# boundless-xyz/boundless

Measured on AMD Instinct MI355X. Metric: segment-proofs/sec @ 2^20 cycles, higher is better.
Workload: dtype u32 (BabyBear Montgomery)

## Files before the change

### boundless_amd/csrc/poseidon2.hip

```cpp
#include "ctx.hpp"
#include "poseidon2_arith.hpp"
#include "hash_suite.hpp"
#include "../../include/bx_image.h"

namespace bx {

constexpr int CELLS = 24, RATE = 16, RF_HALF = 4, RP = 21;
constexpr int DIAG_OFF = 216;
constexpr int PAIR_OFF = DIAG_OFF + 24, P2_TABLE = PAIR_OFF + 2 * CELLS;

typedef uint32_t sgpr8 __attribute__((ext_vector_type(8)));
static_assert(DIAG_OFF % 8 == 0 && PAIR_OFF % 8 == 0 && CELLS % 8 == 0, "the tables are read as 32-byte octets");
template <int LO = 0, int HI = CELLS>
__device__ __forceinline__ void poseidon2_mix(uint32_t* io, const uint32_t* __restrict__ prm) {
    i32 s[CELLS];
    i64 y[CELLS];
#pragma unroll
    for (int i = 0; i < CELLS; ++i) s[i] = (i32)io[i];
    m_ext64s(s, y);
    redc64s_all(y, prm, s);
#pragma unroll 1
    for (int r = 0; r < RF_HALF; ++r) {
        sbox7s_n<CELLS / 2>(s);
        sbox7s_n<CELLS / 2>(s + CELLS / 2);
        m_ext64s(s, y);
        if (r < RF_HALF - 1) {
            redc64s_all(y, prm + (r + 1) * CELLS, s);
        } else {
            red64ks_all<K1_MID, K2_MID, true>(y, prm[96], s);
        }
    }
    {
        const sgpr8* kp = reinterpret_cast<const sgpr8*>(prm + PAIR_OFF);
        sgpr8 k0 = kp[0], k1 = kp[1], k2 = kp[2], k3 = kp[3], k4 = kp[4], k5 = kp[5];
        asm volatile("" : "+s"(k0), "+s"(k1), "+s"(k2), "+s"(k3), "+s"(k4), "+s"(k5));
        i32 pk[2 * CELLS];
#pragma unroll
        for (int i = 0; i < 8; ++i) {
            pk[i] = (i32)k0[i], pk[8 + i] = (i32)k1[i], pk[16 + i] = (i32)k2[i];
            pk[24 + i] = (i32)k3[i], pk[32 + i] = (i32)k4[i], pk[40 + i] = (i32)k5[i];
        }
#pragma unroll 1
        for (int r = 0; r < RP - 1; r += 2) {
            internal_round_pair(s, pk, pk + CELLS, prm + 97 + r);
        }
    }
    uint32_t diag[CELLS];
    {
        const sgpr8* dp = reinterpret_cast<const sgpr8*>(prm + DIAG_OFF);
        sgpr8 d0 = dp[0], d1 = dp[1], d2 = dp[2];
        asm volatile("" : "+s"(d0), "+s"(d1), "+s"(d2));
#pragma unroll
        for (int i = 0; i < 8; ++i) diag[i] = d0[i], diag[8 + i] = d1[i], diag[16 + i] = d2[i];
    }
    internal_round<true>(s, diag, prm + 117);
    i64 t[4];
#pragma unroll 1
    for (int r = 0;; ++r) {
        sbox7s_n<CELLS / 2>(s);
        sbox7s_n<CELLS / 2>(s + CELLS / 2);
        m_ext64s_core(s, y, t);
        asm volatile("" : "+s"(r));
        if (r == RF_HALF - 1) break;
        m_ext64s_finish(y, t);
        redc64s_all(y, prm + 117 + (r + 1) * CELLS, s);
    }
    m_ext64s_finish<LO, HI>(y, t);
    red64ks_all<K1_END, K2_END, false, LO, HI>(y, 0u, s);
#pragma unroll
    for (int i = LO; i < HI; ++i) io[i] = canon(s[i]);
}

__global__ __launch_bounds__(256) __attribute__((amdgpu_waves_per_eu(4, 4))) void hash_rows_kernel(uint32_t* __restrict__ out, const uint32_t* __restrict__ matrix,
                                                        const uint32_t* __restrict__ prm, uint32_t rows, uint32_t cols) {
    uint32_t r = blockIdx.x * blockDim.x + threadIdx.x;
    if (r >= rows) return;
    uint32_t s[CELLS];
#pragma unroll
    for (int i = 0; i < CELLS; ++i) s[i] = 0u;
    const uint32_t* p = matrix + r;
    uint32_t c = 0;
    for (; c + RATE < cols; c += RATE) {
#pragma unroll
        for (int i = 0; i < RATE; ++i) s[i] = p[(size_t)(c + i) * rows];
        poseidon2_mix<RATE, CELLS>(s, prm);
    }
#pragma unroll
    for (int i = 0; i < RATE; ++i) s[i] = (c + i < cols) ? p[(size_t)(c + i) * rows] : 0u;
    poseidon2_mix<0, 8>(s, prm);
    uint4* o = reinterpret_cast<uint4*>(out + (size_t)r * 8);
    o[0] = make_uint4(s[0], s[1], s[2], s[3]);
    o[1] = make_uint4(s[4], s[5], s[6], s[7]);
}

__global__ __launch_bounds__(256) __attribute__((amdgpu_waves_per_eu(4, 4))) void hash_fold_kernel(uint32_t* __restrict__ io, const uint32_t* __restrict__ prm,
                                                        uint32_t input_size, uint32_t output_size) {
    uint32_t i = blockIdx.x * blockDim.x + threadIdx.x;
    if (i >= output_size) return;
    const uint4* src = reinterpret_cast<const uint4*>(io + ((size_t)input_size + 2 * (size_t)i) * 8);
    uint32_t s[CELLS];
    uint4 v0 = src[0], v1 = src[1], v2 = src[2], v3 = src[3];
    s[0] = v0.x; s[1] = v0.y; s[2] = v0.z; s[3] = v0.w;
    s[4] = v1.x; s[5] = v1.y; s[6] = v1.z; s[7] = v1.w;
    s[8] = v2.x; s[9] = v2.y; s[10] = v2.z; s[11] = v2.w;
    s[12] = v3.x; s[13] = v3.y; s[14] = v3.z; s[15] = v3.w;
#pragma unroll
    for (int k = 16; k < CELLS; ++k) s[k] = 0u;
    poseidon2_mix<0, 8>(s, prm);
    uint4* o = reinterpret_cast<uint4*>(io + ((size_t)output_size + i) * 8);
    o[0] = make_uint4(s[0], s[1], s[2], s[3]);
    o[1] = make_uint4(s[4], s[5], s[6], s[7]);
}

__global__ __launch_bounds__(256) __attribute__((amdgpu_waves_per_eu(4, 4))) void hash_fold_indexed_kernel(uint32_t* out, const uint32_t* in,
                                                                const uint32_t* __restrict__ sel, const uint32_t* __restrict__ prm,
                                                                uint32_t count, uint32_t n_in) {
    uint32_t j = blockIdx.x * blockDim.x + threadIdx.x;
    if (j >= count) return;
    uint2 pr = reinterpret_cast<const uint2*>(sel)[j];
    pr.x = pr.x < n_in ? pr.x : n_in - 1;
    pr.y = pr.y < n_in ? pr.y : n_in - 1;
    const uint4* a = reinterpret_cast<const uint4*>(in + (size_t)pr.x * 8);
    const uint4* b = reinterpret_cast<const uint4*>(in + (size_t)pr.y * 8);
    uint32_t s[CELLS];
    uint4 v0 = a[0], v1 = a[1], v2 = b[0], v3 = b[1];
    s[0] = v0.x; s[1] = v0.y; s[2] = v0.z; s[3] = v0.w;
    s[4] = v1.x; s[5] = v1.y; s[6] = v1.z; s[7] = v1.w;
    s[8] = v2.x; s[9] = v2.y; s[10] = v2.z; s[11] = v2.w;
    s[12] = v3.x; s[13] = v3.y; s[14] = v3.z; s[15] = v3.w;
#pragma unroll
    for (int k = 16; k < CELLS; ++k) s[k] = 0u;
    poseidon2_mix<0, 8>(s, prm);
    uint4* o = reinterpret_cast<uint4*>(out + (size_t)j * 8);
    o[0] = make_uint4(s[0], s[1], s[2], s[3]);
    o[1] = make_uint4(s[4], s[5], s[6], s[7]);
}

__device__ __forceinline__ void fold_pair(uint32_t* out8, const uint32_t* a8, const uint32_t* b8, const uint32_t* __restrict__ prm) {
    uint32_t s[CELLS];
#pragma unroll
    for (int k = 0; k < 8; ++k) s[k] = a8[k], s[8 + k] = b8[k];
#pragma unroll
    for (int k = 16; k < CELLS; ++k) s[k] = 0u;
    uint32_t z;
    asm volatile("s_mov_b32 %0, 0" : "=s"(z));
    poseidon2_mix<0, 8>(s, prm + z);
#pragma unroll
    for (int k = 0; k < 8; ++k) out8[k] = s[k];
}
__device__ __forceinline__ void ld_digest(uint32_t* d, const uint32_t* p) {
    const uint4 a = reinterpret_cast<const uint4*>(p)[0], b = reinterpret_cast<const uint4*>(p)[1];
    d[0] = a.x; d[1] = a.y; d[2] = a.z; d[3] = a.w; d[4] = b.x; d[5] = b.y; d[6] = b.z; d[7] = b.w;
}
__device__ __forceinline__ void st_digest(uint32_t* p, const uint32_t* d) {
    reinterpret_cast<uint4*>(p)[0] = make_uint4(d[0], d[1], d[2], d[3]);
    reinterpret_cast<uint4*>(p)[1] = make_uint4(d[4], d[5], d[6], d[7]);
}
template <int LVL>
__device__ __forceinline__ void fold_subtree(uint32_t* out8, uint32_t* __restrict__ io, const uint32_t* __restrict__ prm, size_t input_size, size_t idx) {
    uint32_t a[8], b[8];
    if constexpr (LVL == 1) {
        ld_digest(a, io + (input_size + 2 * idx) * 8);
        ld_digest(b, io + (input_size + 2 * idx + 1) * 8);
    } else {
        fold_subtree<LVL - 1>(a, io, prm, input_size, 2 * idx);
        fold_subtree<LVL - 1>(b, io, prm, input_size, 2 * idx + 1);
    }
    fold_pair(out8, a, b, prm);
// ... 153 lines not shown
        sbox7s_n<QS>(s);
        m_ext_quad(s, y, m);
        if (r < RF_HALF - 1) redc_quad(y, shp + 117 + (r + 1) * CELLS + q, s);
        else redk_quad<K1_END, K2_END>(y, 0u, s);
    }
#pragma unroll
    for (int k = 0; k < QS; ++k) io[k] = canon(s[k]);
}

__global__ __launch_bounds__(1024) void hash_fold_quad_kernel(uint32_t* __restrict__ io, const uint32_t* __restrict__ prm, uint32_t input_size,
                                                              uint32_t per_wg, int levels) {
    __shared__ uint32_t sh[256 * 8];
    __shared__ uint32_t shp[DIAG_OFF + 24];
    const uint32_t tid = threadIdx.x, q = tid & 3, node = tid >> 2;
    for (uint32_t i = tid; i < DIAG_OFF + 24; i += blockDim.x) shp[i] = prm[i];
    uint32_t width = per_wg >> 1;
    uint32_t out_size = input_size >> 1;
    for (int lvl = 0; lvl < levels; ++lvl) {
        const bool active = node < width;
        uint32_t s[QS];
        if (active) {
            if (lvl == 0) {
                const uint32_t* src = io + ((size_t)input_size + 2 * ((size_t)blockIdx.x * width + node)) * 8;
#pragma unroll
                for (int k = 0; k < 4; ++k) s[k] = src[4 * k + q];
            } else {
#pragma unroll
                for (int k = 0; k < 4; ++k) s[k] = sh[node * 16 + 4 * k + q];
            }
            s[4] = 0u;
            s[5] = 0u;
        }
        __syncthreads();
        if (active) {
            poseidon2_mix_quad(s, shp, q);
            uint32_t* o = io + ((size_t)out_size + (size_t)blockIdx.x * width + node) * 8;
            o[q] = s[0];
            o[4 + q] = s[1];
            sh[node * 8 + q] = s[0];
            sh[node * 8 + 4 + q] = s[1];
        }
        __syncthreads();
        width >>= 1;
        out_size >>= 1;
    }
}

__global__ __launch_bounds__(64) void transcript_step_kernel(uint32_t* __restrict__ state, const uint32_t* __restrict__ digests, uint32_t n_commit,
                                                            uint32_t* __restrict__ out, uint32_t n_elems, const uint32_t* __restrict__ prm) {
    __shared__ uint32_t shp[DIAG_OFF + 24];
    const uint32_t tid = threadIdx.x, q = tid & 3;
    for (uint32_t i = tid; i < DIAG_OFF + 24; i += blockDim.x) shp[i] = prm[i];
    __syncthreads();
    if (tid >= 4) return;
    uint32_t s[QS];
#pragma unroll
    for (int k = 0; k < QS; ++k) s[k] = state[4 * k + q];
    uint32_t pool = state[24];
    for (uint32_t i = 0; i < n_commit; ++i) {
        if (pool != 0) {
            poseidon2_mix_quad(s, shp, q);
            pool = 0;
        }
        s[0] = fp_add(s[0], digests[8 * i + q]);
        s[1] = fp_add(s[1], digests[8 * i + 4 + q]);
        poseidon2_mix_quad(s, shp, q);
    }
    for (uint32_t e = 0; e < n_elems; ++e) {
        if (pool == 16) {
            poseidon2_mix_quad(s, shp, q);
            pool = 0;
        }
        const uint32_t slot = pool >> 2;
        const uint32_t v = slot == 0 ? s[0] : slot == 1 ? s[1] : slot == 2 ? s[2] : s[3];
        if ((pool & 3u) == q) out[e] = v;
        ++pool;
    }
#pragma unroll
    for (int k = 0; k < QS; ++k) state[4 * k + q] = s[k];
    if (q == 0) state[24] = pool;
}

const char* poseidon2_upload_params(bx_ctx* c) {
    uint32_t h[P2_TABLE] = {0};
    for (int i = 0; i < 213; ++i) h[i] = (uint32_t)((uint64_t)(c->h_rc[i] % P) * p2_rc_scale(i) % P);
    for (int i = 0; i < 24; ++i) h[DIAG_OFF + i] = fp_encode(c->h_diag[i]);
    i32 pe[CELLS], pa[CELLS];
    p2_pair_consts(h + DIAG_OFF, pe, pa);
    for (int i = 0; i < CELLS; ++i) h[PAIR_OFF + i] = (uint32_t)pe[i], h[PAIR_OFF + CELLS + i] = (uint32_t)pa[i];
    if (!c->d_p2) BX_HIP(c, hipMalloc(&c->d_p2, sizeof h));
    BX_HIP(c, hipMemcpyAsync(c->d_p2, h, sizeof h, hipMemcpyHostToDevice, c->stream));
    BX_HIP(c, stream_wait(c));
    return nullptr;
}

static const char* launch_hash_rows(bx_ctx* c, uint32_t* out, const uint32_t* matrix, size_t rows, size_t cols) {
    if (rows == 0) return nullptr;
    unsigned bs = (unsigned)c->hash_rows_block;
    hipLaunchKernelGGL(hash_rows_kernel, dim3((unsigned)((rows + bs - 1) / bs)), dim3(bs), 0, c->stream, out, matrix, c->d_p2,
                       (uint32_t)rows, (uint32_t)cols);
    BX_LAUNCH_CHECK(c);
    return nullptr;
}
static const char* launch_hash_fold(bx_ctx* c, uint32_t* io, size_t input_size, size_t output_size) {
    if (output_size == 0) return nullptr;
    hipLaunchKernelGGL(hash_fold_kernel, dim3((unsigned)((output_size + 255) / 256)), dim3(256), 0, c->stream, io, c->d_p2,
                       (uint32_t)input_size, (uint32_t)output_size);
    BX_LAUNCH_CHECK(c);
    return nullptr;
}
template <int L>
static const char* launch_hash_fold_deep(bx_ctx* c, uint32_t* io, size_t size) {
    hipLaunchKernelGGL(hash_fold_deep_kernel<L>, dim3((unsigned)(((size >> L) + 255) / 256)), dim3(256), 0, c->stream, io, c->d_p2, (uint32_t)size);
    BX_LAUNCH_CHECK(c);
    return nullptr;
}
static const char* launch_hash_fold_small(bx_ctx* c, uint32_t* io, size_t size, size_t per_wg, int levels) {
    if (c->fold_quad)
        hipLaunchKernelGGL(hash_fold_quad_kernel, dim3((unsigned)(size / per_wg)), dim3((unsigned)(2 * per_wg)), 0, c->stream, io, c->d_p2,
                           (uint32_t)size, (uint32_t)per_wg, levels);
    else
        hipLaunchKernelGGL(hash_fold_multi_kernel, dim3((unsigned)(size / per_wg)), dim3(256), 0, c->stream, io, c->d_p2, (uint32_t)size,
                           (uint32_t)per_wg, levels);
    BX_LAUNCH_CHECK(c);
    return nullptr;
}
HashLaunchers poseidon2_launchers() { return {launch_hash_rows, launch_hash_fold, launch_hash_fold_deep<3>, launch_hash_fold_deep<2>, launch_hash_fold_small}; }

}

using namespace bx;

extern "C" const char* bx_poseidon2_set_params(bx_ctx* c, const uint32_t* rc213, const uint32_t* diag24) try {
    if (!c) return "bx_poseidon2_set_params: null ctx";
    BX_REQUIRE(c, rc213 && diag24, "poseidon2_set_params: null table");
    BX_REQUIRE(c, c->live_provers == 0, "poseidon2_set_params: destroy the provers of this ctx first (their transcripts hold the old table)");
    BX_ENTER(c);
    for (int i = 0; i < 213; ++i) c->h_rc[i] = rc213[i] % P;
    for (int i = 0; i < 24; ++i) c->h_diag[i] = diag24[i] % P;
    return poseidon2_upload_params(c);
} BX_ABI_CATCH(c, "bx_poseidon2_set_params")
extern "C" const char* bx_poseidon2_get_params(bx_ctx* c, uint32_t* rc213, uint32_t* diag24) try {
    if (!c) return "bx_poseidon2_get_params: null ctx";
    for (int i = 0; i < 213; ++i) rc213[i] = c->h_rc[i];
    for (int i = 0; i < 24; ++i) diag24[i] = c->h_diag[i];
    return nullptr;
} BX_ABI_CATCH(c, "bx_poseidon2_get_params")

extern "C" const char* bx_hash_fold_indexed(bx_ctx* c, bx_buf out, bx_buf in, bx_buf sel, size_t count) try {
    if (!c) return "bx_hash_fold_indexed: null ctx";
    BX_REQUIRE(c, count <= out.len / 8 && count <= sel.len / 2, "hash_fold_indexed: out or sel too small");
    BX_REQUIRE(c, count <= 0xffffffffu && in.len / 8 <= 0xffffffffu, "hash_fold_indexed: too many digests");
    if (count == 0) return nullptr;
    BX_REQUIRE(c, out.dptr && in.dptr && sel.dptr && in.len >= 8, "hash_fold_indexed: null or empty buffer");
    BX_REQUIRE(c, !bufs_overlap(out, in), "hash_fold_indexed: out and in overlap");
    BX_REQUIRE(c, !bufs_overlap(out, sel), "hash_fold_indexed: out and sel overlap");
    BX_ENTER(c);
    OpScope op(c, "hash_fold_indexed", 104.0 * (double)count);
    hipLaunchKernelGGL(hash_fold_indexed_kernel, dim3((unsigned)((count + 255) / 256)), dim3(256), 0, c->stream, (uint32_t*)out.dptr,
                       (const uint32_t*)in.dptr, (const uint32_t*)sel.dptr, c->d_p2, (uint32_t)count, (uint32_t)(in.len / 8));
    BX_LAUNCH_CHECK(c);
    return nullptr;
} BX_ABI_CATCH(c, "bx_hash_fold_indexed")

extern "C" const char* bx_transcript_step(bx_ctx* c, bx_buf state, bx_buf digests, size_t n_commit, bx_buf out_ext, size_t n_ext) try {
    if (!c) return "bx_transcript_step: null ctx";
    BX_REQUIRE(c, c->hash_suite == SUITE_POSEIDON2, "transcript_step: the device transcript is Poseidon2's (a sha-256 ctx draws on the host)");
    BX_REQUIRE(c, state.dptr != nullptr && state.len >= 25, "transcript_step: the state is 24 cells and the pool counter");
    BX_REQUIRE(c, n_commit <= 64 && n_ext <= 64, "transcript_step: at most 64 commits and 64 challenges per step");
    BX_REQUIRE(c, digests.len >= 8 * n_commit && out_ext.len >= 4 * n_ext, "transcript_step: digests / out too small");
    BX_REQUIRE(c, !bufs_overlap(out_ext, state), "transcript_step: out_ext and state overlap");
    BX_REQUIRE(c, !bufs_overlap(out_ext, digests), "transcript_step: out_ext and digests overlap");
// ... 9 lines not shown
```

### boundless_amd/csrc/poseidon2_arith.hpp

```cpp
#pragma once
#include "fp.hpp"

#if defined(BX_CHECK_BOUNDS) && !defined(__HIP_DEVICE_COMPILE__)
#include <stdio.h>
#include <stdlib.h>
#define BX_ASSERT_BOUND(cond, what)                                              \
    do {                                                                         \
        if (!(cond)) {                                                           \
            fprintf(stderr, "bound violated: %s (%s:%d)\n", what, __FILE__, __LINE__); \
            abort();                                                             \
        }                                                                        \
    } while (0)
#else
#define BX_ASSERT_BOUND(cond, what) ((void)0)
#endif

#if defined(BX_PLAIN_MAD)
#define BX_MAD_FLAVOUR mad_plain
#else
#define BX_MAD_FLAVOUR mad_pinned
#endif
namespace bx {
inline namespace BX_MAD_FLAVOUR {

constexpr int P2_CELLS = 24;

constexpr uint32_t cx_mul(uint32_t a, uint32_t b) { return (uint32_t)((uint64_t)a * b % P); }
constexpr uint32_t cx_pow(uint32_t b, uint64_t e) {
    uint32_t r = 1;
    while (e) {
        if (e & 1) r = cx_mul(r, b);
        b = cx_mul(b, b);
        e >>= 1;
    }
    return r;
}
constexpr uint32_t cx_rpow(int64_t e) { return cx_pow(MONT_ONE, e >= 0 ? (uint64_t)e : (uint64_t)((int64_t)(P - 1) + e)); }
constexpr uint32_t K1_MID = cx_rpow(2801), K2_MID = cx_mul(K1_MID, MONT_ONE);
constexpr uint32_t K1_END = cx_rpow(400), K2_END = cx_mul(K1_END, MONT_ONE);
constexpr uint32_t p2_rc_scale(int i) {
    return i < 24 ? cx_rpow(1) : i < 48 ? cx_rpow(-6) : i < 72 ? cx_rpow(-55) : i < 96 ? cx_rpow(-398)
         : i < 141 ? cx_rpow(2)
         : i < 165 ? cx_rpow(1) : i < 189 ? cx_rpow(-6) : cx_rpow(-55);
}

using i32 = int32_t;
using i64 = int64_t;
constexpr i64 SREDC_MAX = ((i64)0x7fffffff - (i64)(P / 2) - 2) * ((i64)1 << 32);

#if defined(__HIP_DEVICE_COMPILE__) && !defined(BX_PLAIN_MAD)
#define BX_MAD_ASM(op, args, ...)                                                                  \
    do {                                                                                           \
        switch (alt & 3) {                                                                         \
            case 0: asm volatile(op " %0, s[40:41], " args : "=v"(r) : __VA_ARGS__ : "s40", "s41"); break; \
            case 1: asm volatile(op " %0, s[42:43], " args : "=v"(r) : __VA_ARGS__ : "s42", "s43"); break; \
            case 2: asm volatile(op " %0, s[44:45], " args : "=v"(r) : __VA_ARGS__ : "s44", "s45"); break; \
            default: asm volatile(op " %0, s[46:47], " args : "=v"(r) : __VA_ARGS__ : "s46", "s47"); break; \
        }                                                                                          \
    } while (0)
#endif
BX_HD i64 smad(i32 a, i32 b, i64 c, int alt = 0) {
#if defined(__HIP_DEVICE_COMPILE__) && !defined(BX_PLAIN_MAD)
    i64 r;
    BX_MAD_ASM("v_mad_i64_i32", "%1, %2, %3", "v"(a), "v"(b), "v"(c));
    return r;
#else
    (void)alt;
    return (i64)a * (i64)b + c;
#endif
}
BX_HD i64 smul(i32 a, i32 b, int alt = 0) {
#if defined(__HIP_DEVICE_COMPILE__) && !defined(BX_PLAIN_MAD)
    i64 r;
    BX_MAD_ASM("v_mad_i64_i32", "%1, %2, 0", "v"(a), "v"(b));
    return r;
#else
    (void)alt;
    return (i64)a * (i64)b;
#endif
}
BX_HD i64 smad_k(i32 a, uint32_t k, i64 c, int alt = 0) {
#if defined(__HIP_DEVICE_COMPILE__) && !defined(BX_PLAIN_MAD)
    i64 r;
    BX_MAD_ASM("v_mad_i64_i32", "%1, %2, %3", "v"(a), "s"(k), "v"(c));
    return r;
#else
    (void)alt;
    return (i64)a * (i64)k + c;
#endif
}
BX_HD i64 smul_k(i32 a, uint32_t k, int alt = 0) {
#if defined(__HIP_DEVICE_COMPILE__) && !defined(BX_PLAIN_MAD)
    i64 r;
    BX_MAD_ASM("v_mad_i64_i32", "%1, %2, 0", "v"(a), "s"(k));
    return r;
#else
    (void)alt;
    return (i64)a * (i64)k;
#endif
}
BX_HD i64 smad_s(i32 a, i32 k, i64 c, int alt = 0) {
#if defined(__HIP_DEVICE_COMPILE__) && !defined(BX_PLAIN_MAD)
    i64 r;
    BX_MAD_ASM("v_mad_i64_i32", "%1, %2, %3", "v"(a), "s"(k), "v"(c));
    return r;
#else
    (void)alt;
    return (i64)a * (i64)k + c;
#endif
}
BX_HD i64 smul_s(i32 a, i32 k, int alt = 0) {
#if defined(__HIP_DEVICE_COMPILE__) && !defined(BX_PLAIN_MAD)
    i64 r;
    BX_MAD_ASM("v_mad_i64_i32", "%1, %2, 0", "v"(a), "s"(k));
    return r;
#else
    (void)alt;
    return (i64)a * (i64)k;
#endif
}
template <int K>
BX_HD i64 smadc(i32 a, i64 c, int alt = 0) {
#if defined(__HIP_DEVICE_COMPILE__) && !defined(BX_PLAIN_MAD)
    i64 r;
    BX_MAD_ASM("v_mad_i64_i32", "%1, %3, %2", "v"(a), "v"(c), "n"(K));
    return r;
#else
    (void)alt;
    return (i64)a * K + c;
#endif
}
template <int K>
BX_HD i64 smulc(i32 a, int alt = 0) {
#if defined(__HIP_DEVICE_COMPILE__) && !defined(BX_PLAIN_MAD)
    i64 r;
    BX_MAD_ASM("v_mad_i64_i32", "%1, %2, 0", "v"(a), "n"(K));
    return r;
#else
    (void)alt;
    return (i64)a * K;
#endif
}
BX_HD i64 add_u32(i64 c, uint32_t k, int alt = 0) {
#if defined(__HIP_DEVICE_COMPILE__) && !defined(BX_PLAIN_MAD)
    i64 r;
    BX_MAD_ASM("v_mad_u64_u32", "%1, 1, %2", "s"(k), "v"(c));
    return r;
#else
    (void)alt;
    return c + (i64)k;
#endif
}
BX_HD i64 umul_k(uint32_t a, uint32_t k, int alt = 0) {
#if defined(__HIP_DEVICE_COMPILE__) && !defined(BX_PLAIN_MAD)
    i64 r;
    BX_MAD_ASM("v_mad_u64_u32", "%1, %2, 0", "v"(a), "s"(k));
    return r;
#else
    (void)alt;
    return (i64)((uint64_t)a * (uint64_t)k);
#endif
}
BX_HD i32 mont_m(i64 t) {
#if defined(__HIP_DEVICE_COMPILE__) && !defined(BX_PLAIN_MAD)
    i32 m;
    asm volatile("v_mul_lo_u32 %0, %1, %2" : "=v"(m) : "v"((uint32_t)t), "s"(NEG_P_INV));
    return m;
#else
    return (i32)((uint32_t)t * NEG_P_INV);
#endif
}
BX_HD i32 sredc(i64 t, int alt = 0) {
    BX_ASSERT_BOUND(t <= SREDC_MAX && t >= -SREDC_MAX, "sredc operand");
    const i32 m = mont_m(t);
    return (i32)(smad_k(m, P, t, alt) >> 32);
}
BX_HD i64 iabs64(i64 v) { return v < 0 ? -v : v; }

constexpr i64 ub(i64 T) { return (T >> 32) + (i64)(P / 2) + 1; }
constexpr i64 B_IN = (i64)P - 1;
constexpr i64 B_Y = 112 * ((i64)1 << 31);
constexpr i64 B_EXT = ub(B_Y + (i64)P);
constexpr i64 B_MIDOUT = ub(((i64)1 << 32) * K1_MID + ((B_Y >> 32) + 1) * (i64)K2_MID + 2 * (i64)P);
constexpr i64 B_SUMR = ub(((i64)1 << 31) * R2 + 33 * (i64)R3);
constexpr i64 B_INT = (i64)((double)P * 0.945);
static_assert(ub((i64)(P - 1) * B_INT + B_SUMR + (i64)P) <= B_INT && B_MIDOUT <= B_INT, "internal-round bound is not invariant");
static_assert((i64)(P - 1) * B_INT + B_SUMR + (i64)P <= SREDC_MAX && B_INT * B_INT <= SREDC_MAX, "internal-round products overflow sredc");
static_assert(24 * B_INT < ((i64)1 << 37), "internal sum");

BX_HD uint64_t mad64(uint32_t a, uint32_t b, uint64_t c) { return (uint64_t)a * (uint64_t)b + c; }

template <int N>
BX_HD void sredc_n(const i64* t, i32* r) {
    i32 m[N];
#pragma unroll
    for (int i = 0; i < N; ++i) {
        BX_ASSERT_BOUND(t[i] <= SREDC_MAX && t[i] >= -SREDC_MAX, "sredc operand");
        m[i] = mont_m(t[i]);
    }
#pragma unroll
    for (int i = 0; i < N; ++i) r[i] = (i32)(smad_k(m[i], P, t[i], i & 3) >> 32);
}

BX_HD i32 sbox7s(i32 x) {
    BX_ASSERT_BOUND(iabs64(x) <= B_INT, "sbox input");
    const i32 x2 = sredc(smul(x, x));
    const i32 x3 = sredc(smul(x2, x));
    const i32 x4 = sredc(smul(x2, x2));
    return sredc(smul(x3, x4));
}
template <int N>
BX_HD void sbox7s_n(i32* x) {
    i64 t[N], u[N];
    i32 x2[N], x3[N], x4[N];
#pragma unroll
    for (int i = 0; i < N; ++i) {
        BX_ASSERT_BOUND(iabs64(x[i]) <= B_INT, "sbox input");
        t[i] = smul(x[i], x[i], i & 3);
    }
    sredc_n<N>(t, x2);
#pragma unroll
    for (int i = 0; i < N; ++i) {
        t[i] = smul(x2[i], x[i], 2 * i);
        u[i] = smul(x2[i], x2[i], 2 * i + 1);
    }
    sredc_n<N>(t, x3);
    sredc_n<N>(u, x4);
#pragma unroll
    for (int i = 0; i < N; ++i) t[i] = smul(x3[i], x4[i], i & 3);
    sredc_n<N>(t, x);
}

BX_HD i32 redc64s(i64 y, uint32_t rc) {
    BX_ASSERT_BOUND(iabs64(y) <= B_Y, "external layer output");
    const i32 r = sredc(add_u32(y, rc));
    BX_ASSERT_BOUND(iabs64(r) <= B_EXT, "redc64s output");
    return r;
}

BX_HD void redc64s_all(const i64* y, const uint32_t* rc, i32* s) {
    constexpr int H = P2_CELLS / 2;
#pragma unroll
    for (int h = 0; h < P2_CELLS; h += H) {
        i64 acc[H];
#pragma unroll
        for (int i = 0; i < H; ++i) {
            BX_ASSERT_BOUND(iabs64(y[h + i]) <= B_Y, "external layer output");
            acc[i] = add_u32(y[h + i], rc[h + i], i & 3);
        }
        sredc_n<H>(acc, s + h);
    }
#pragma unroll
    for (int i = 0; i < P2_CELLS; ++i) BX_ASSERT_BOUND(iabs64(s[i]) <= B_EXT, "redc64s output");
}

template <uint32_t K1, uint32_t K2, bool HAS_ADD = true>
BX_HD i32 red64ks(i64 y, uint32_t add) {
    BX_ASSERT_BOUND(iabs64(y) <= B_Y, "external layer output");
    static_assert(K1 < (1u << 29) && K2 < P, "correction constant too large for the accumulator bound");
    i64 acc = umul_k((uint32_t)y, K1);
    if (HAS_ADD) acc = add_u32(acc, add);
    return sredc(smad_k((i32)(y >> 32), K2, acc));
}
template <uint32_t K1, uint32_t K2, bool HAS_ADD0, int LO = 0, int HI = P2_CELLS>
BX_HD void red64ks_all(const i64* y, uint32_t add0, i32* s) {
    static_assert(K1 < (1u << 29) && K2 < P, "correction constant too large for the accumulator bound");
    static_assert(0 <= LO && LO < HI && HI <= P2_CELLS && (!HAS_ADD0 || LO == 0), "live range");
    constexpr int H = HI - LO < P2_CELLS / 2 ? HI - LO : P2_CELLS / 2;
    static_assert((HI - LO) % H == 0, "live range: a whole number of stages");
#pragma unroll
    for (int h = LO; h < HI; h += H) {
        i64 acc[H];
#pragma unroll
        for (int i = 0; i < H; ++i) {
            BX_ASSERT_BOUND(iabs64(y[h + i]) <= B_Y, "external layer output");
            acc[i] = umul_k((uint32_t)y[h + i], K1, i & 3);
        }
        if (HAS_ADD0 && h == 0) acc[0] = add_u32(acc[0], add0, 0);
#pragma unroll
        for (int i = 0; i < H; ++i) acc[i] = smad_k((i32)(y[h + i] >> 32), K2, acc[i], (i + 1) & 3);
        sredc_n<H>(acc, s + h);
    }
}

BX_HD void m_ext64s_core(const i32* s, i64* y, i64* t) {
#pragma unroll
    for (int h = 0; h < 2; ++h) {
        i64 t0[3], t1[3], t2[3], t3[3];
#pragma unroll
        for (int q = 0; q < 3; ++q) {
            const int g = 3 * h + q;
            t0[q] = smulc<1>(s[4 * g], 2 * q);
            t1[q] = smulc<1>(s[4 * g + 2], 2 * q + 1);
        }
#pragma unroll
        for (int q = 0; q < 3; ++q) {
            const int g = 3 * h + q;
            t0[q] = smadc<1>(s[4 * g + 1], t0[q], 2 * q + 2);
            t1[q] = smadc<1>(s[4 * g + 3], t1[q], 2 * q + 3);
        }
#pragma unroll
        for (int q = 0; q < 3; ++q) {
            const int g = 3 * h + q;
            t2[q] = smadc<2>(s[4 * g + 1], t1[q], 2 * q);
            t3[q] = smadc<2>(s[4 * g + 3], t0[q], 2 * q + 1);
        }
#pragma unroll
        for (int q = 0; q < 3; ++q) {
            const int g = 3 * h + q;
            const i64 t4 = t1[q] * 4 + t3[q], t5 = t0[q] * 4 + t2[q];
            y[4 * g] = t3[q] + t5;
            y[4 * g + 1] = t5;
            y[4 * g + 2] = t2[q] + t4;
            y[4 * g + 3] = t4;
        }
    }
#pragma unroll
    for (int j = 0; j < 4; ++j) {
        t[j] = y[j];
#pragma unroll
        for (int k = 4; k < P2_CELLS; k += 4) t[j] += y[k + j];
    }
}
template <int LO = 0, int HI = P2_CELLS>
BX_HD void m_ext64s_finish(i64* y, const i64* t) {
    static_assert(0 <= LO && LO < HI && HI <= P2_CELLS, "live range");
#pragma unroll
    for (int i = LO; i < HI; ++i) y[i] += t[i & 3];
}
BX_HD void m_ext64s(const i32* s, i64* y) {
    i64 t[4];
    m_ext64s_core(s, y, t);
    m_ext64s_finish(y, t);
}

BX_HD i32 internal_sum_rs(i64 sum) {
// ... 124 lines not shown
    i64 a0 = smul_s(x0, E[0], 2);
    i64 f = fold64(sum1, 3);
    gx = smad_s(s[2], A[2], gx, 0);
    m = mont_m(f);
    gy = smad_s(s[6], A[6], gy, 1);
    const i32 sig1 = (i32)(smad_k(m, P, f, 2) >> 32);
    BX_ASSERT_BOUND(iabs64(sig1) <= B_SIG1, "sig1");
    gx = smad_s(s[3], A[3], gx, 3);
    gy = smad_s(s[7], A[7], gy, 0);
    a0 = smad_k(sig1, R2, a0, 1);
    gx = smad_s(s[4], A[4], gx, 2);
    a0 = add_u32(a0, rc[0], 3);
    BX_ASSERT_BOUND(iabs64(a0) <= T_PAIR0, "cell 0, round A");
    gy = smad_s(s[8], A[8], gy, 0);
    m = mont_m(a0);
    gx = smad_s(sig1, K23R3, gx, 1);
    const i32 y0 = (i32)(smad_k(m, P, a0, 2) >> 32);
    BX_ASSERT_BOUND(iabs64(y0) <= B_INT && iabs64(gx) <= T_DOT && iabs64(gy) <= T_DOT, "sbox input");
    i64 fx = fold64(gx, 3);
    t = smul(y0, y0, 0);
    i64 fy = fold64(gy, 1);
    gx = smad_s(s[9], A[9], fx, 2);
    m = mont_m(t);
    gy = smad_s(s[13], A[13], fy, 3);
    x2 = (i32)(smad_k(m, P, t, 0) >> 32);
    gx = smad_s(s[10], A[10], gx, 1);
    gy = smad_s(s[14], A[14], gy, 2);
    t = smul(x2, y0, 3);
    gx = smad_s(s[11], A[11], gx, 0);
    u = smul(x2, x2, 1);
    gy = smad_s(s[15], A[15], gy, 2);
    m = mont_m(t);
    gx = smad_s(s[12], A[12], gx, 3);
    m2 = mont_m(u);
    gy = smad_s(s[16], A[16], gy, 0);
    x3 = (i32)(smad_k(m, P, t, 1) >> 32);
    BX_ASSERT_BOUND(iabs64(gx) <= T_DOT && iabs64(gy) <= T_DOT, "dot-product group");
    fx = fold64(gx, 2);
    x4 = (i32)(smad_k(m2, P, u, 3) >> 32);
    fy = fold64(gy, 0);
    t = smul(x3, x4, 1);
    gx = smad_s(s[17], A[17], fx, 2);
    gx = smad_s(s[18], A[18], gx, 3);
    m = mont_m(t);
    gx = smad_s(s[19], A[19], gx, 0);
    gx = smad_s(s[20], A[20], gx, 1);
    const i32 y0s = (i32)(smad_k(m, P, t, 2) >> 32);
    BX_ASSERT_BOUND(iabs64(gx) <= T_DOT && iabs64(y0s) <= B_SBOX, "dot-product group");
    fx = fold64(gx, 3);
    gy = smad_s(s[21], A[21], fy, 0);
    gy = smad_s(s[22], A[22], gy, 1);
    gy = smad_s(s[23], A[23], gy, 2);
    gy = smad_k(y0s, R2, gy + fx, 3);
    BX_ASSERT_BOUND(iabs64(gy) <= T_LAST, "last dot-product group");
    const i32 sig2 = sredc(fold64(gy, 0), 1);
    BX_ASSERT_BOUND(iabs64(sig2) <= B_SIG2, "sig2");
    const i64 c = smulc<1>(sig2, 2);
    constexpr int H = P2_CELLS / 2;
#pragma unroll
    for (int h = 0; h < P2_CELLS; h += H) {
        i64 tt[H];
#pragma unroll
        for (int i = 0; i < H; ++i) {
            if (h + i == 0)
                tt[i] = smad_s(y0s, E[0], add_u32(c, rc[1], 2), 3);
            else
                tt[i] = smad_s(s[h + i], E[h + i], c, i + 2);
        }
#pragma unroll
        for (int i = 0; i < H; ++i)
            if (h + i != 0) tt[i] = smad_s(sig1, A[h + i], tt[i], i + 1);
        sredc_n<H>(tt, s + h);
    }
#pragma unroll
    for (int i = 0; i < P2_CELLS; ++i) BX_ASSERT_BOUND(iabs64(s[i]) <= B_INT, "internal cell");
}

BX_HD uint32_t canon(i32 v) {
    BX_ASSERT_BOUND(iabs64(v) < (i64)P, "canonicalisation input");
    const uint32_t u = (uint32_t)v;
    return umin(u, u + P);
}

template <int DIAG, int LO = 0, int HI = P2_CELLS>
BX_HD void poseidon2_mix_bounded(uint32_t* io, const uint32_t* prm) {
    i32 s[P2_CELLS];
    i64 y[P2_CELLS];
    const uint32_t* diag = prm + DIAG;
    for (int i = 0; i < P2_CELLS; ++i) {
        BX_ASSERT_BOUND(io[i] <= B_IN, "canonical input");
        s[i] = (i32)io[i];
    }
    m_ext64s(s, y);
    redc64s_all(y, prm, s);
    for (int r = 0; r < 4; ++r) {
        sbox7s_n<P2_CELLS>(s);
        m_ext64s(s, y);
        if (r < 3) {
            redc64s_all(y, prm + (r + 1) * P2_CELLS, s);
        } else {
            red64ks_all<K1_MID, K2_MID, true>(y, prm[96], s);
            for (int i = 0; i < P2_CELLS; ++i) BX_ASSERT_BOUND(iabs64(s[i]) <= B_MIDOUT, "mid transition output");
        }
    }
    i32 pair_e[P2_CELLS], pair_a[P2_CELLS];
    p2_pair_consts(diag, pair_e, pair_a);
    for (int r = 0; r < 20; r += 2) internal_round_pair(s, pair_e, pair_a, prm + 97 + r);
    internal_round<true>(s, diag, prm + 117);
    for (int r = 0; r < 4; ++r) {
        i64 t[4];
        sbox7s_n<P2_CELLS>(s);
        m_ext64s_core(s, y, t);
        if (r < 3) {
            m_ext64s_finish(y, t);
            redc64s_all(y, prm + 117 + (r + 1) * P2_CELLS, s);
        } else {
            m_ext64s_finish<LO, HI>(y, t);
            red64ks_all<K1_END, K2_END, false, LO, HI>(y, 0u, s);
            for (int i = LO; i < HI; ++i) io[i] = canon(s[i]);
        }
    }
}

}
}
```

Before: 32.53.

## Fold external-round constants through MDS inverse into S-box final multiply

Precomputes, on the host, round constants pulled back through the inverse of the external linear layer. Each full-round S-box then adds them inside its last multiply-add (v_mad_i64_i32 with a scalar addend), and the separate constant add before reduction becomes a plain sredc. Capacity cells between absorb blocks in hash_rows are carried signed rather than canonicalised, saving the canon ops. This adds a larger parameter table and a host-side check that the folded constants reproduce the originals, and relies on the new bounds analysis being correct.

```diff
diff --git a/boundless_amd/csrc/poseidon2.hip b/boundless_amd/csrc/poseidon2.hip
--- a/boundless_amd/csrc/poseidon2.hip
+++ b/boundless_amd/csrc/poseidon2.hip
@@ -6,13 +6,25 @@
 namespace bx {
 
 constexpr int CELLS = 24, RATE = 16, RF_HALF = 4, RP = 21;
-constexpr int DIAG_OFF = 216;
-constexpr int PAIR_OFF = DIAG_OFF + 24, P2_TABLE = PAIR_OFF + 2 * CELLS;
+constexpr int DIAG_OFF = P2_DIAG_OFF;
+constexpr int PAIR_OFF = P2_PAIR_OFF;
+constexpr int FOLD_OFF = P2_FOLD_OFF, P2_TABLE = P2_TABLE_WORDS;
 
 typedef uint32_t sgpr8 __attribute__((ext_vector_type(8)));
-static_assert(DIAG_OFF % 8 == 0 && PAIR_OFF % 8 == 0 && CELLS % 8 == 0, "the tables are read as 32-byte octets");
-template <int LO = 0, int HI = CELLS>
+typedef uint64_t sgpr4q __attribute__((ext_vector_type(4)));
+static_assert(DIAG_OFF % 8 == 0 && PAIR_OFF % 8 == 0 && FOLD_OFF % 8 == 0 && CELLS % 8 == 0, "the tables are read as 32-byte octets");
+__device__ __forceinline__ void sbox_half_folded(i32* s, const uint32_t* __restrict__ prm, int block, int h) {
+    const sgpr4q* fp = reinterpret_cast<const sgpr4q*>(prm + FOLD_OFF + block * P2_FOLD_BLOCK + h * CELLS);
+    sgpr4q f0 = fp[0], f1 = fp[1], f2 = fp[2];
+    asm volatile("" : "+s"(f0), "+s"(f1), "+s"(f2));
+    i64 K[CELLS / 2];
+#pragma unroll
+    for (int i = 0; i < 4; ++i) K[i] = (i64)f0[i], K[4 + i] = (i64)f1[i], K[8 + i] = (i64)f2[i];
+    sbox7s_n<CELLS / 2>(s + h * (CELLS / 2), K);
+}
+template <int LO = 0, int HI = CELLS, bool SIGNED = false>
 __device__ __forceinline__ void poseidon2_mix(uint32_t* io, const uint32_t* __restrict__ prm) {
+    static_assert(!SIGNED || LO >= RATE, "only capacity cells are carried signed");
     i32 s[CELLS];
     i64 y[CELLS];
 #pragma unroll
@@ -21,11 +33,12 @@
     redc64s_all(y, prm, s);
 #pragma unroll 1
     for (int r = 0; r < RF_HALF; ++r) {
-        sbox7s_n<CELLS / 2>(s);
-        sbox7s_n<CELLS / 2>(s + CELLS / 2);
+        asm volatile("" : "+s"(r));
+        sbox_half_folded(s, prm, r, 0);
+        sbox_half_folded(s, prm, r, 1);
         m_ext64s(s, y);
         if (r < RF_HALF - 1) {
-            redc64s_all(y, prm + (r + 1) * CELLS, s);
+            sredc_all(y, s);
         } else {
             red64ks_all<K1_MID, K2_MID, true>(y, prm[96], s);
         }
@@ -57,18 +70,18 @@
     i64 t[4];
 #pragma unroll 1
     for (int r = 0;; ++r) {
-        sbox7s_n<CELLS / 2>(s);
-        sbox7s_n<CELLS / 2>(s + CELLS / 2);
+        asm volatile("" : "+s"(r));
+        sbox_half_folded(s, prm, RF_HALF + r, 0);
+        sbox_half_folded(s, prm, RF_HALF + r, 1);
         m_ext64s_core(s, y, t);
-        asm volatile("" : "+s"(r));
         if (r == RF_HALF - 1) break;
         m_ext64s_finish(y, t);
-        redc64s_all(y, prm + 117 + (r + 1) * CELLS, s);
+        sredc_all(y, s);
     }
     m_ext64s_finish<LO, HI>(y, t);
     red64ks_all<K1_END, K2_END, false, LO, HI>(y, 0u, s);
 #pragma unroll
-    for (int i = LO; i < HI; ++i) io[i] = canon(s[i]);
+    for (int i = LO; i < HI; ++i) io[i] = SIGNED ? (uint32_t)s[i] : canon(s[i]);
 }
 
 __global__ __launch_bounds__(256) __attribute__((amdgpu_waves_per_eu(4, 4))) void hash_rows_kernel(uint32_t* __restrict__ out, const uint32_t* __restrict__ matrix,
@@ -83,7 +96,7 @@
     for (; c + RATE < cols; c += RATE) {
 #pragma unroll
         for (int i = 0; i < RATE; ++i) s[i] = p[(size_t)(c + i) * rows];
-        poseidon2_mix<RATE, CELLS>(s, prm);
+        poseidon2_mix<RATE, CELLS, true>(s, prm);
     }
 #pragma unroll
     for (int i = 0; i < RATE; ++i) s[i] = (c + i < cols) ? p[(size_t)(c + i) * rows] : 0u;
@@ -403,12 +416,8 @@
 }
 
 const char* poseidon2_upload_params(bx_ctx* c) {
-    uint32_t h[P2_TABLE] = {0};
-    for (int i = 0; i < 213; ++i) h[i] = (uint32_t)((uint64_t)(c->h_rc[i] % P) * p2_rc_scale(i) % P);
-    for (int i = 0; i < 24; ++i) h[DIAG_OFF + i] = fp_encode(c->h_diag[i]);
-    i32 pe[CELLS], pa[CELLS];
-    p2_pair_consts(h + DIAG_OFF, pe, pa);
-    for (int i = 0; i < CELLS; ++i) h[PAIR_OFF + i] = (uint32_t)pe[i], h[PAIR_OFF + CELLS + i] = (uint32_t)pa[i];
+    uint32_t h[P2_TABLE];
+    if (!p2_build_table(c->h_rc, c->h_diag, h)) return "poseidon2_upload_params: the folded round constants do not reproduce the stored ones";
     if (!c->d_p2) BX_HIP(c, hipMalloc(&c->d_p2, sizeof h));
     BX_HIP(c, hipMemcpyAsync(c->d_p2, h, sizeof h, hipMemcpyHostToDevice, c->stream));
     BX_HIP(c, stream_wait(c));
diff --git a/boundless_amd/csrc/poseidon2_arith.hpp b/boundless_amd/csrc/poseidon2_arith.hpp
--- a/boundless_amd/csrc/poseidon2_arith.hpp
+++ b/boundless_amd/csrc/poseidon2_arith.hpp
@@ -79,6 +79,16 @@
     return (i64)a * (i64)b;
 #endif
 }
+BX_HD i64 smad_c64(i32 a, i32 b, i64 c, int alt = 0) {
+#if defined(__HIP_DEVICE_COMPILE__) && !defined(BX_PLAIN_MAD)
+    i64 r;
+    BX_MAD_ASM("v_mad_i64_i32", "%1, %2, %3", "v"(a), "v"(b), "s"(c));
+    return r;
+#else
+    (void)alt;
+    return (i64)a * (i64)b + c;
+#endif
+}
 BX_HD i64 smad_k(i32 a, uint32_t k, i64 c, int alt = 0) {
 #if defined(__HIP_DEVICE_COMPILE__) && !defined(BX_PLAIN_MAD)
     i64 r;
@@ -209,8 +219,12 @@
     const i32 x4 = sredc(smul(x2, x2));
     return sredc(smul(x3, x4));
 }
-template <int N>
-BX_HD void sbox7s_n(i32* x) {
+constexpr i64 B_X2 = ub(B_INT * B_INT), B_X3 = ub(B_X2 * B_INT), B_X4 = ub(B_X2 * B_X2);
+constexpr i64 T_SBOX_K = B_X3 * B_X4 + (i64)P - 1;
+constexpr i64 B_SBOX_K = ub(T_SBOX_K);
+static_assert(T_SBOX_K <= SREDC_MAX && B_SBOX_K <= ub(B_X3 * B_X4) + 1 && B_SBOX_K <= B_INT, "S-box with a folded constant leaves its bounds");
+template <int N, bool HAS_K>
+BX_HD void sbox7s_stages(i32* x, const i64* K) {
     i64 t[N], u[N];
     i32 x2[N], x3[N], x4[N];
 #pragma unroll
@@ -227,9 +241,25 @@
     sredc_n<N>(t, x3);
     sredc_n<N>(u, x4);
 #pragma unroll
-    for (int i = 0; i < N; ++i) t[i] = smul(x3[i], x4[i], i & 3);
+    for (int i = 0; i < N; ++i) {
+        if constexpr (HAS_K) {
+            BX_ASSERT_BOUND(K[i] >= 0 && K[i] < (i64)P, "folded round constant");
+            t[i] = smad_c64(x3[i], x4[i], K[i], i & 3);
+            BX_ASSERT_BOUND(iabs64(t[i]) <= T_SBOX_K, "sbox last product");
+        } else {
+            t[i] = smul(x3[i], x4[i], i & 3);
+        }
+    }
     sredc_n<N>(t, x);
-}
+    if constexpr (HAS_K) {
+#pragma unroll
+        for (int i = 0; i < N; ++i) BX_ASSERT_BOUND(iabs64(x[i]) <= B_SBOX_K, "sbox output");
+    }
+}
+template <int N>
+BX_HD void sbox7s_n(i32* x) { sbox7s_stages<N, false>(x, nullptr); }
+template <int N>
+BX_HD void sbox7s_n(i32* x, const i64* K) { sbox7s_stages<N, true>(x, K); }
 
 BX_HD i32 redc64s(i64 y, uint32_t rc) {
     BX_ASSERT_BOUND(iabs64(y) <= B_Y, "external layer output");
@@ -252,6 +282,16 @@
     }
 #pragma unroll
     for (int i = 0; i < P2_CELLS; ++i) BX_ASSERT_BOUND(iabs64(s[i]) <= B_EXT, "redc64s output");
+}
+
+BX_HD void sredc_all(const i64* y, i32* s) {
+    constexpr int H = P2_CELLS / 2;
+#pragma unroll
+    for (int i = 0; i < P2_CELLS; ++i) BX_ASSERT_BOUND(iabs64(y[i]) <= B_Y, "external layer output");
+#pragma unroll
+    for (int h = 0; h < P2_CELLS; h += H) sredc_n<H>(y + h, s + h);
+#pragma unroll
+    for (int i = 0; i < P2_CELLS; ++i) BX_ASSERT_BOUND(iabs64(s[i]) <= B_EXT, "sredc_all output");
 }
 
 template <uint32_t K1, uint32_t K2, bool HAS_ADD = true>
@@ -542,22 +582,141 @@
     return umin(u, u + P);
 }
 
-template <int DIAG, int LO = 0, int HI = P2_CELLS>
+constexpr int P2_RC_WORDS = 213, P2_DIAG_OFF = 216, P2_PAIR_OFF = P2_DIAG_OFF + P2_CELLS, P2_FOLD_OFF = P2_PAIR_OFF + 2 * P2_CELLS;
+constexpr int P2_FOLD_BLOCK = 2 * P2_CELLS, P2_FOLD_BLOCKS = 8, P2_FOLD_WORDS = P2_FOLD_BLOCKS * P2_FOLD_BLOCK;
+constexpr int P2_TABLE_WORDS = P2_FOLD_OFF + P2_FOLD_WORDS;
+static_assert(P2_DIAG_OFF % 8 == 0 && P2_PAIR_OFF % 8 == 0 && P2_FOLD_OFF % 8 == 0 && (P2_FOLD_BLOCK / 2) % 8 == 0, "the tables are read as 32-byte octets");
+
+struct P2M4 {
+    uint32_t a[4][4];
+};
+constexpr uint32_t cx_sub(uint32_t a, uint32_t b) { return a >= b ? a - b : a + P - b; }
+constexpr P2M4 P2_M4 = {{{5, 7, 1, 3}, {4, 6, 1, 1}, {1, 3, 5, 7}, {1, 1, 4, 6}}};
+constexpr P2M4 p2_m4_mul(const P2M4& x, const P2M4& y) {
+    P2M4 r = {};
+    for (int i = 0; i < 4; ++i)
+        for (int j = 0; j < 4; ++j) {
+            uint32_t v = 0;
+            for (int k = 0; k < 4; ++k) v = (uint32_t)(((uint64_t)x.a[i][k] * y.a[k][j] + v) % P);
+            r.a[i][j] = v;
+        }
+    return r;
+}
+constexpr P2M4 p2_m4_inverse() {
+    uint32_t m[4][8] = {};
+    for (int i = 0; i < 4; ++i) {
+        for (int j = 0; j < 4; ++j) m[i][j] = P2_M4.a[i][j];
+        m[i][4 + i] = 1;
+    }
+    for (int col = 0; col < 4; ++col) {
+        int p = col;
+        while (p < 3 && m[p][col] == 0) ++p;
+        for (int j = 0; j < 8; ++j) {
+            const uint32_t v = m[p][j];
+            m[p][j] = m[col][j];
+            m[col][j] = v;
+        }
+        const uint32_t inv = cx_pow(m[col][col], P - 2);
+        for (int j = 0; j < 8; ++j) m[col][j] = cx_mul(m[col][j], inv);
+        for (int i = 0; i < 4; ++i) {
+            if (i == col) continue;
+            const uint32_t f = m[i][col];
+            for (int j = 0; j < 8; ++j) m[i][j] = cx_sub(m[i][j], cx_mul(f, m[col][j]));
+        }
+    }
+    P2M4 r = {};
+    for (int i = 0; i < 4; ++i)
+        for (int j = 0; j < 4; ++j) r.a[i][j] = m[i][4 + j];
+    return r;
+}
+constexpr bool p2_m4_is_identity(const P2M4& x) {
+    for (int i = 0; i < 4; ++i)
+        for (int j = 0; j < 4; ++j)
+            if (x.a[i][j] != (i == j ? 1u : 0u)) return false;
+    return true;
+}
+static_assert(p2_m4_is_identity(p2_m4_mul(P2_M4, p2_m4_inverse())), "M4^-1");
+
+BX_HD const uint32_t* p2_fold_source(const uint32_t* prm, int b) {
+    return (b & 3) == 3 ? nullptr : b < 3 ? prm + (b + 1) * P2_CELLS : prm + 117 + (b - 3) * P2_CELLS;
+}
+BX_HD bool p2_fold_consts(const uint32_t* prm, uint32_t* fold) {
+    constexpr P2M4 inv = p2_m4_inverse();
+    constexpr uint32_t inv7 = cx_pow(7u, P - 2);
+    bool ok = true;
+    for (int b = 0; b < P2_FOLD_BLOCKS; ++b) {
+        uint32_t* out = fold + b * P2_FOLD_BLOCK;
+        for (int i = 0; i < P2_FOLD_BLOCK; ++i) out[i] = 0u;
+        const uint32_t* rc = p2_fold_source(prm, b);
+        if (!rc) continue;
+        uint32_t c[P2_CELLS], seventh[4], t[4] = {0u, 0u, 0u, 0u};
+        for (int j = 0; j < 4; ++j) {
+            uint64_t sum = 0;
+            for (int k = 0; k < P2_CELLS; k += 4) sum += rc[k + j] % P;
+            seventh[j] = (uint32_t)(sum % P * inv7 % P);
+        }
+        for (int k = 0; k < P2_CELLS; k += 4)
+            for (int i = 0; i < 4; ++i) {
+                uint64_t v = 0;
+                for (int j = 0; j < 4; ++j) v = ((uint64_t)inv.a[i][j] * ((rc[k + j] % P + P - seventh[j]) % P) + v) % P;
+                c[k + i] = (uint32_t)v;
+            }
+        uint32_t w[P2_CELLS];
+        for (int k = 0; k < P2_CELLS; k += 4)
+            for (int i = 0; i < 4; ++i) {
+                uint64_t v = 0;
+                for (int j = 0; j < 4; ++j) v += (uint64_t)P2_M4.a[i][j] * c[k + j];
+                w[k + i] = (uint32_t)(v % P);
+                t[i] = (uint32_t)(((uint64_t)t[i] + w[k + i]) % P);
+            }
+        for (int i = 0; i < P2_CELLS; ++i) {
+            ok = ok && (uint32_t)(((uint64_t)w[i] + t[i & 3]) % P) == rc[i] % P;
+            out[2 * i] = (uint32_t)((uint64_t)c[i] * MONT_ONE % P);
+        }
+    }
+    return ok;
+}
+BX_HD void p2_fold_half(const uint32_t* fold, int b, int h, i64* K) {
+    const uint32_t* f = fold + b * P2_FOLD_BLOCK + h * P2_CELLS;
+    for (int i = 0; i < P2_CELLS / 2; ++i) K[i] = (i64)(((uint64_t)f[2 * i + 1] << 32) | f[2 * i]);
+}
+BX_HD bool p2_build_table(const uint32_t* rc213, const uint32_t* diag24, uint32_t* table) {
+    for (int i = 0; i < P2_TABLE_WORDS; ++i) table[i] = 0u;
+    for (int i = 0; i < P2_RC_WORDS; ++i) table[i] = (uint32_t)((uint64_t)(rc213[i] % P) * p2_rc_scale(i) % P);
+    for (int i = 0; i < P2_CELLS; ++i) table[P2_DIAG_OFF + i] = fp_encode(diag24[i]);
+    i32 pe[P2_CELLS], pa[P2_CELLS];
+    p2_pair_consts(table + P2_DIAG_OFF, pe, pa);
+    for (int i = 0; i < P2_CELLS; ++i) table[P2_PAIR_OFF + i] = (uint32_t)pe[i], table[P2_PAIR_OFF + P2_CELLS + i] = (uint32_t)pa[i];
+    return p2_fold_consts(table, table + P2_FOLD_OFF);
+}
+
+constexpr i64 B_CARRY = (i64)K1_END + (i64)(P / 2) + 60;
+static_assert(B_CARRY < (i64)P, "carried capacity cells");
+template <int DIAG, int LO = 0, int HI = P2_CELLS, bool SIGNED_OUT = false>
 BX_HD void poseidon2_mix_bounded(uint32_t* io, const uint32_t* prm) {
+    static_assert(!SIGNED_OUT || LO >= 16, "only capacity cells are carried signed");
     i32 s[P2_CELLS];
-    i64 y[P2_CELLS];
+    i64 y[P2_CELLS], K[P2_CELLS / 2];
     const uint32_t* diag = prm + DIAG;
     for (int i = 0; i < P2_CELLS; ++i) {
-        BX_ASSERT_BOUND(io[i] <= B_IN, "canonical input");
+        if (i < 16) BX_ASSERT_BOUND(io[i] <= B_IN, "canonical input");
+        else BX_ASSERT_BOUND(iabs64((i32)io[i]) <= B_IN, "capacity input: canonical or carried signed");
         s[i] = (i32)io[i];
     }
+    uint32_t fold[P2_FOLD_WORDS];
+    const bool folded = p2_fold_consts(prm, fold);
+    BX_ASSERT_BOUND(folded, "M c == rc' for the folded rounds");
+    (void)folded;
     m_ext64s(s, y);
     redc64s_all(y, prm, s);
     for (int r = 0; r < 4; ++r) {
-        sbox7s_n<P2_CELLS>(s);
+        for (int h = 0; h < 2; ++h) {
+            p2_fold_half(fold, r, h, K);
+            sbox7s_n<P2_CELLS / 2>(s + h * (P2_CELLS / 2), K);
+        }
         m_ext64s(s, y);
         if (r < 3) {
-            redc64s_all(y, prm + (r + 1) * P2_CELLS, s);
+            sredc_all(y, s);
         } else {
             red64ks_all<K1_MID, K2_MID, true>(y, prm[96], s);
             for (int i = 0; i < P2_CELLS; ++i) BX_ASSERT_BOUND(iabs64(s[i]) <= B_MIDOUT, "mid transition output");
@@ -569,18 +728,28 @@
     internal_round<true>(s, diag, prm + 117);
     for (int r = 0; r < 4; ++r) {
         i64 t[4];
-        sbox7s_n<P2_CELLS>(s);
+        for (int h = 0; h < 2; ++h) {
+            p2_fold_half(fold, 4 + r, h, K);
+            sbox7s_n<P2_CELLS / 2>(s + h * (P2_CELLS / 2), K);
+        }
         m_ext64s_core(s, y, t);
         if (r < 3) {
             m_ext64s_finish(y, t);
-            redc64s_all(y, prm + 117 + (r + 1) * P2_CELLS, s);
+            sredc_all(y, s);
         } else {
             m_ext64s_finish<LO, HI>(y, t);
             red64ks_all<K1_END, K2_END, false, LO, HI>(y, 0u, s);
-            for (int i = LO; i < HI; ++i) io[i] = canon(s[i]);
-        }
-    }
-}
-
-}
-}
+            for (int i = LO; i < HI; ++i) {
+                if (SIGNED_OUT) {
+                    BX_ASSERT_BOUND(iabs64(s[i]) <= B_CARRY, "carried capacity cell");
+                    io[i] = (uint32_t)s[i];
+                } else {
+                    io[i] = canon(s[i]);
+                }
+            }
+        }
+    }
+}
+
+}
+}
```

After: 33.05 (median of 6 runs). 1.02x the previous value.
